# MILab-PKU/dcpt

Measured on AMD Instinct MI355X. Metric: megapixels/sec fwd+bwd NAFNet-64 256px bs=32, higher is better.
Workload: dtype f32

## Files before the change

dcpt_amd/csrc/ffn_f32.h:

```cpp
#pragma once
#include "dcpt_common.h"

struct FfnFwdF {
    const float* y;
    const float *lnw, *lnb;
    const float *W4, *W5;
    const float *b4, *b5, *gamma;
    float* out;
    float* v;
    float *mu, *rstd;
    int64_t M;
    float eps;
};
bool ffn_fwd_f32_ok(int C);
int launch_ffn_fwd_f32(const FfnFwdF& p, int C, hipStream_t s);
int launch_ln_conv_f32(const FfnFwdF& p, int C, hipStream_t s);

struct FfnBwdF {
    const float *dout, *v, *y;
    const float *wT5, *wT4;
    const float* lnw;
    float *dv, *dy;
    float* lnpart;
    int64_t M;
    float eps;
};
int ffn_bwd_f32_waves(int64_t M);
int launch_ffn_bwd_f32(const FfnBwdF& p, int C, hipStream_t s);
```

dcpt_amd/csrc/ffn_f32.hip:

```cpp
#include "bufops.h"
#include "ffn_f32.h"

namespace {

#ifdef F32_ABL_NOMFMA
#define FFN_MFMA(a, b, c) (c)
#else
#define FFN_MFMA(a, b, c) __builtin_amdgcn_mfma_f32_32x32x2f32(a, b, c, 0, 0, 0)
#endif

constexpr int FW = 4;
constexpr int S_SLOT = 8192, S_RING = 4, S_WAVE = S_RING * S_SLOT;
constexpr int S_TAB = FW * S_WAVE;
constexpr int T_B4 = 0, T_B5 = 128, T_GM = 192, T_LW = 256, T_LB = 320, T_N = 384;

__device__ __forceinline__ void lds_fence() { asm volatile("s_waitcnt lgkmcnt(0)" ::: "memory"); }

template <int C, int HEAD>
__global__ __launch_bounds__(256) void ffn_fwd_f32_kernel(const FfnFwdF p) {
    static_assert(C == 64, "ffn_fwd_f32: C = 64");
    __shared__ __attribute__((aligned(16))) unsigned char smem[S_TAB + T_N * 4];
    const int tid = threadIdx.x, lane = tid & 63;
    const int wave = __builtin_amdgcn_readfirstlane(tid >> 6);
    float* const tab = reinterpret_cast<float*>(smem + S_TAB);
    for (int i = tid; i < T_N; i += 256)
        tab[i] = i < T_B5 ? (p.b4 ? p.b4[i] : 0.f)
                          : i < T_LW ? (HEAD ? 0.f : (i < T_GM ? (p.b5 ? p.b5[i - T_B5] : 0.f) : (p.gamma ? p.gamma[i - T_GM] : 1.f)))
                                     : i < T_LB ? p.lnw[i - T_LW] : p.lnb[i - T_LB];
    const int fr = lane & 31, kh = lane >> 5;
    float W4f[4][32], W5f[2][32];
#pragma unroll
    for (int j = 0; j < 4; ++j)
#pragma unroll
        for (int q = 0; q < 8; ++q) {
// ... 113 lines not shown
#pragma unroll
            for (int j = 0; j < 2; ++j)
#pragma unroll
                for (int g = 0; g < 4; ++g) {
                    const float4 b = *reinterpret_cast<const float4*>(tab + T_B5 + 32 * j + 8 * g + 4 * kh);
                    acc2[j][4 * g + 0] = b.x; acc2[j][4 * g + 1] = b.y; acc2[j][4 * g + 2] = b.z; acc2[j][4 * g + 3] = b.w;
                }
#pragma unroll
            for (int ks = 0; ks < 32; ++ks)
#pragma unroll
                for (int j = 0; j < 2; ++j) acc2[j] = FFN_MFMA(W5f[j][ks], xf[ks], acc2[j]);
            const rsrc_t rsO = make_rsrc(p.out + r0 * C);
#pragma unroll
            for (int j = 0; j < 2; ++j)
#pragma unroll
                for (int g = 0; g < 4; ++g) {
                    const float4 gm = *reinterpret_cast<const float4*>(tab + T_GM + 32 * j + 8 * g + 4 * kh);
                    const float4 yv = yres[4 * j + g];
                    buf_st4(rsO, rowok ? (uint32_t)(fr * 256 + (8 * j + 2 * g + kh) * 16) : ROW_SENT,
                            make_float4(yv.x + acc2[j][4 * g + 0] * gm.x, yv.y + acc2[j][4 * g + 1] * gm.y, yv.z + acc2[j][4 * g + 2] * gm.z,
                                        yv.w + acc2[j][4 * g + 3] * gm.w));
                }
        }
        lds_fence();
        asm volatile("s_waitcnt vmcnt(16)" ::: "memory");
        s = (s + 1) & 3;
    }
    dma_wait_all();
}


constexpr int G_DO = 0, G_V = 4096, G_Y = 12288, G_SLOT = 16384, G_WAVE = 2 * G_SLOT;
constexpr int G_TAB = FW * G_WAVE;
typedef float floatx4v __attribute__((ext_vector_type(4)));

template <int C>
__global__ __launch_bounds__(256) void ffn_bwd_f32_kernel(const FfnBwdF p) {
    static_assert(C == 64, "ffn_bwd_f32: C = 64");
    __shared__ __attribute__((aligned(16))) unsigned char smem[G_TAB + 64 * 4];
    const int tid = threadIdx.x, lane = tid & 63;
    const int wave = __builtin_amdgcn_readfirstlane(tid >> 6);
    float* const tab = reinterpret_cast<float*>(smem + G_TAB);
    if (tid < 64) tab[tid] = p.lnw[tid];
    const int fm = lane & 15, q = lane >> 4;
    float W5f[4][16], W4f[4][32];
#pragma unroll
    for (int t = 0; t < 4; ++t) {
#pragma unroll
        for (int e = 0; e < 4; ++e) {
            const float4 w = ldg4(p.wT5 + (16 * t + fm) * C + 16 * q + 4 * e);
            W5f[t][4 * e + 0] = w.x; W5f[t][4 * e + 1] = w.y; W5f[t][4 * e + 2] = w.z; W5f[t][4 * e + 3] = w.w;
        }
#pragma unroll
        for (int e = 0; e < 8; ++e) {
            const float4 w = ldg4(p.wT4 + (16 * t + fm) * (2 * C) + 32 * q + 4 * e);
            W4f[t][4 * e + 0] = w.x; W4f[t][4 * e + 1] = w.y; W4f[t][4 * e + 2] = w.z; W4f[t][4 * e + 3] = w.w;
        }
    }
    __syncthreads();

    unsigned char* const wb = smem + wave * G_WAVE;
    const uint32_t wb_lds = lds_addr(reinterpret_cast<const float*>(wb));
    const int64_t ng = (p.M + 15) / 16;
    const int64_t wg = (int64_t)blockIdx.x * FW + wave, TW = (int64_t)gridDim.x * FW;
    auto issue = [&](int64_t gi, int s) {
        const int64_t gg = gi < ng ? gi : 0;
        const i32x4 rsD = make_rsrc_dma(p.dout + gg * (16 * C)), rsY = make_rsrc_dma(p.y + gg * (16 * C)), rsV = make_rsrc_dma(p.v + gg * (32 * C));
        const uint32_t base = wb_lds + (uint32_t)(s * G_SLOT);
#pragma unroll
        for (int pc = 0; pc < 4; ++pc) {
            const int row = 4 * pc + (lane >> 4);
            const bool ok = gi < ng && gi * 16 + row < p.M;
            const uint32_t vo = ok ? (uint32_t)(row * 256 + (((lane & 15) ^ (row & 15)) * 16)) : ROW_SENT;
            dma16(rsD, base + (uint32_t)(G_DO + pc * 1024), vo, 0);
            dma16(rsY, base + (uint32_t)(G_Y + pc * 1024), vo, 0);
        }
#pragma unroll
        for (int pc = 0; pc < 8; ++pc) {
            const int row = 2 * pc + (lane >> 5);
            const bool ok = gi < ng && gi * 16 + row < p.M;
            dma16(rsV, base + (uint32_t)(G_V + pc * 1024), ok ? (uint32_t)(row * 512 + (((lane & 31) ^ (row & 15)) * 16)) : ROW_SENT, 0);
        }
    };
    issue(wg, 0);
    issue(wg + TW, 1);
    asm volatile("s_waitcnt vmcnt(16)" ::: "memory");

    float aw[4][4], ab[4][4];
#pragma unroll
    for (int t = 0; t < 4; ++t)
#pragma unroll
        for (int r = 0; r < 4; ++r) aw[t][r] = ab[t][r] = 0.f;

    int s = 0;
    for (int64_t gi = wg; gi < ng; gi += TW) {
        unsigned char* const sl = wb + s * G_SLOT;
        const int sw = fm;
        float xb[32];
#pragma unroll
        for (int e = 0; e < 4; ++e) {
            const float4 w = *reinterpret_cast<const float4*>(sl + G_DO + fm * 256 + (((4 * q + e) ^ sw) * 16));
            xb[4 * e + 0] = w.x; xb[4 * e + 1] = w.y; xb[4 * e + 2] = w.z; xb[4 * e + 3] = w.w;
        }
        floatx4v dg[4];
#pragma unroll
        for (int t = 0; t < 4; ++t) dg[t] = floatx4v{0.f, 0.f, 0.f, 0.f};
#pragma unroll
        for (int st = 0; st < 16; ++st)
#pragma unroll
            for (int t = 0; t < 4; ++t) dg[t] = __builtin_amdgcn_mfma_f32_16x16x4f32(W5f[t][st], xb[st], dg[t], 0, 0, 0);
#pragma unroll
        for (int t = 0; t < 4; ++t) {
            float4* const a1 = reinterpret_cast<float4*>(sl + G_V + fm * 512 + (((4 * t + q) ^ sw) * 16));
            float4* const a2 = reinterpret_cast<float4*>(sl + G_V + fm * 512 + (((16 + 4 * t + q) ^ sw) * 16));
            const float4 v1 = *a1, v2 = *a2;
            const float4 d = make_float4(dg[t][0], dg[t][1], dg[t][2], dg[t][3]);
            *a1 = f4_mul(d, v2);
            *a2 = f4_mul(d, v1);
        }
        lds_fence();
#pragma unroll
        for (int e = 0; e < 8; ++e) {
            const float4 w = *reinterpret_cast<const float4*>(sl + G_V + fm * 512 + (((8 * q + e) ^ sw) * 16));
            xb[4 * e + 0] = w.x; xb[4 * e + 1] = w.y; xb[4 * e + 2] = w.z; xb[4 * e + 3] = w.w;
        }
        floatx4v dx[4];
#pragma unroll
        for (int t = 0; t < 4; ++t) dx[t] = floatx4v{0.f, 0.f, 0.f, 0.f};
#pragma unroll
        for (int st = 0; st < 32; ++st)
#pragma unroll
            for (int t = 0; t < 4; ++t) dx[t] = __builtin_amdgcn_mfma_f32_16x16x4f32(W4f[t][st], xb[st], dx[t], 0, 0, 0);
        float xh[4][4];
        float sum = 0.f;
#pragma unroll
        for (int t = 0; t < 4; ++t) {
            const float4 yv = *reinterpret_cast<const float4*>(sl + G_Y + fm * 256 + (((4 * t + q) ^ sw) * 16));
            xh[t][0] = yv.x; xh[t][1] = yv.y; xh[t][2] = yv.z; xh[t][3] = yv.w;
            sum += (yv.x + yv.y) + (yv.z + yv.w);
        }
        sum += __shfl_xor(sum, 16);
        sum += __shfl_xor(sum, 32);
        const float mean = sum * (1.0f / C);
        float sq = 0.f;
#pragma unroll
        for (int t = 0; t < 4; ++t)
#pragma unroll
            for (int r = 0; r < 4; ++r) {
                xh[t][r] -= mean;
                sq += xh[t][r] * xh[t][r];
            }
        sq += __shfl_xor(sq, 16);
        sq += __shfl_xor(sq, 32);
        const float rs = 1.0f / sqrtf(sq * (1.0f / C) + p.eps);
        const bool rowok = gi * 16 + fm < p.M;
        float s1 = 0.f, s2 = 0.f;
        float gwv[4][4];
#pragma unroll
        for (int t = 0; t < 4; ++t) {
            const float4 lw = *reinterpret_cast<const float4*>(tab + 16 * t + 4 * q);
            const float lws[4] = {lw.x, lw.y, lw.z, lw.w};
#pragma unroll
            for (int r = 0; r < 4; ++r) {
                xh[t][r] *= rs;
                const float gx = dx[t][r];
                aw[t][r] += rowok ? gx * xh[t][r] : 0.f;
                ab[t][r] += rowok ? gx : 0.f;
                const float gw = gx * lws[r];
                gwv[t][r] = gw;
                s1 += gw;
                s2 += gw * xh[t][r];
            }
        }
        s1 += __shfl_xor(s1, 16); s1 += __shfl_xor(s1, 32);
        s2 += __shfl_xor(s2, 16); s2 += __shfl_xor(s2, 32);
        s1 *= (1.0f / C);
        s2 *= (1.0f / C);
#pragma unroll
        for (int t = 0; t < 4; ++t) {
            float4* const a = reinterpret_cast<float4*>(sl + G_DO + fm * 256 + (((4 * t + q) ^ sw) * 16));
            const float4 dres = *a;
            *a = make_float4(rs * (gwv[t][0] - xh[t][0] * s2 - s1) + dres.x, rs * (gwv[t][1] - xh[t][1] * s2 - s1) + dres.y,
                             rs * (gwv[t][2] - xh[t][2] * s2 - s1) + dres.z, rs * (gwv[t][3] - xh[t][3] * s2 - s1) + dres.w);
        }
        lds_fence();
        u32x4 ody[4], odv[8];
#pragma unroll
        for (int it = 0; it < 4; ++it) {
            const int row = it * 4 + (lane >> 4), ch = lane & 15;
            ody[it] = *reinterpret_cast<const u32x4*>(sl + G_DO + row * 256 + ((ch ^ (row & 15)) * 16));
        }
#pragma unroll
        for (int it = 0; it < 8; ++it) {
            const int row = it * 2 + (lane >> 5), ch = lane & 31;
            odv[it] = *reinterpret_cast<const u32x4*>(sl + G_V + row * 512 + ((ch ^ (row & 15)) * 16));
        }
        lds_fence();
        issue(gi + 2 * TW, s);
        asm volatile("s_waitcnt vmcnt(16)" ::: "memory");
        const int64_t r0 = gi * 16;
        const rsrc_t rsO = make_rsrc(p.dy + r0 * C), rsV = make_rsrc(p.dv + r0 * (2 * C));
#pragma unroll
        for (int it = 0; it < 4; ++it) {
            const int row = it * 4 + (lane >> 4), ch = lane & 15;
            __builtin_amdgcn_raw_buffer_store_b128(ody[it], rsO, r0 + row < p.M ? (uint32_t)(row * 256 + ch * 16) : ROW_SENT, 0, 0);
        }
#pragma unroll
        for (int it = 0; it < 8; ++it) {
            const int row = it * 2 + (lane >> 5), ch = lane & 31;
            __builtin_amdgcn_raw_buffer_store_b128(odv[it], rsV, r0 + row < p.M ? (uint32_t)(row * 512 + ch * 16) : ROW_SENT, 0, 0);
        }
        s ^= 1;
    }
    dma_wait_all();
#pragma unroll
    for (int t = 0; t < 4; ++t)
#pragma unroll
        for (int r = 0; r < 4; ++r) {
            float a = aw[t][r], b = ab[t][r];
#pragma unroll
            for (int m = 1; m < 16; m <<= 1) {
                a += __shfl_xor(a, m);
                b += __shfl_xor(b, m);
            }
            if (fm == 0) {
                const int c = 16 * t + 4 * q + r;
                p.lnpart[(wg * 2 + 0) * C + c] = a;
                p.lnpart[(wg * 2 + 1) * C + c] = b;
            }
        }
}

}

bool ffn_fwd_f32_ok(int C) { return C == 64; }

static int launch(const FfnFwdF& p, int head, hipStream_t s) {
    int64_t blocks = cdiv64(cdiv64(p.M, 32), FW);
    if (blocks > 256) blocks = 256;
    if (head) ffn_fwd_f32_kernel<64, 1><<<dim3((unsigned)blocks), dim3(256), 0, s>>>(p);
    else ffn_fwd_f32_kernel<64, 0><<<dim3((unsigned)blocks), dim3(256), 0, s>>>(p);
    DCPT_CHECK_LAUNCH("ffn_fwd_f32");
    return DCPT_OK;
}

int launch_ffn_fwd_f32(const FfnFwdF& p, int C, hipStream_t s) {
    DCPT_CHECK_ARG(ffn_fwd_f32_ok(C), "ffn_fwd_f32: C=%d not supported (64)", C);
    DCPT_CHECK_ARG(p.y && p.out && p.W4 && p.W5 && p.lnw && p.lnb && p.M > 0 && (p.mu == nullptr) == (p.rstd == nullptr), "ffn_fwd_f32: null argument");
    return launch(p, 0, s);
}

int launch_ln_conv_f32(const FfnFwdF& p, int C, hipStream_t s) {
    DCPT_CHECK_ARG(ffn_fwd_f32_ok(C), "ln_conv_f32: C=%d not supported (64)", C);
    DCPT_CHECK_ARG(p.y && p.v && p.W4 && p.lnw && p.lnb && p.M > 0 && (p.mu == nullptr) == (p.rstd == nullptr), "ln_conv_f32: null argument");
    return launch(p, 1, s);
}

int ffn_bwd_f32_waves(int64_t M) {
    int64_t blocks = cdiv64(cdiv64(M, 16), FW);
    if (blocks > 256) blocks = 256;
    return (int)blocks * FW;
}

int launch_ffn_bwd_f32(const FfnBwdF& p, int C, hipStream_t s) {
    DCPT_CHECK_ARG(ffn_fwd_f32_ok(C), "ffn_bwd_f32: C=%d not supported (64)", C);
    DCPT_CHECK_ARG(p.dout && p.v && p.y && p.wT5 && p.wT4 && p.lnw && p.dv && p.dy && p.lnpart && p.M > 0, "ffn_bwd_f32: null argument");
    ffn_bwd_f32_kernel<64><<<dim3((unsigned)(ffn_bwd_f32_waves(p.M) / FW)), dim3(256), 0, s>>>(p);
    DCPT_CHECK_LAUNCH("ffn_bwd_f32");
    return DCPT_OK;
}
```

dcpt_amd/csrc/nafblock.hip:

```cpp
#include "gemm.h"
#include "kernels.h"
#include "ffn_f32.h"
#include "side.h"
#include "../../include/dcpt_hip.h"

namespace {

struct FwdWs {
    float* w2p;
    float* pool_part;
    int nblk_pool;
};

size_t fwd_ws_layout(int B, int H, int W, int C, void* base, size_t bytes, FwdWs* out) {
    WsAlloc a(base, base ? bytes : (size_t)-1);
    DwGeom g{B, H, W, C};
    const int nblk = dw_ring_usable(g, 4) ? dw_ring_num_blocks_per_image(g, 4) : dw_num_blocks_per_image(g);
    float* w2p = a.get<float>((size_t)9 * 2 * C);
    float* pp = a.get<float>((size_t)B * nblk * C);
    if (out) {
        out->w2p = w2p;
        out->pool_part = pp;
        out->nblk_pool = nblk;
    }
    return a.off;
}

struct BwdWs {
    float *wT5, *wT4, *wT3, *wT1, *w2p;
    float *b2a, *b2b, *b2c;
    float *bca, *bcb, *bcc;
    float* slab;
    float* colsum;
    size_t slab_elems, colsum_elems;
    float *lnpart, *lnpart2;
    float *ds_part, *ds, *dpool;
    float* wpart;
    int ln_nblk, nblk_b;
    float *u4, *c4, *u1, *c1, *rowpart;
    int rp_sg, rp_dw;
    float* ffn_part;
};

bool ln_in_epilogue(int C);
bool ffn_fused_f32(int C);
size_t bwd_ws_layout(int B, int H, int W, int C, void* base, size_t bytes, BwdWs* out) {
    WsAlloc a(base, base ? bytes : (size_t)-1);
    const int64_t M = (int64_t)B * H * W;
    const int P = H * W;
    DwGeom g{B, H, W, C};
    BwdWs w;
    w.wT5 = a.get<float>((size_t)C * C);
    w.wT4 = a.get<float>((size_t)2 * C * C);
    w.wT3 = a.get<float>((size_t)C * C);
    w.wT1 = a.get<float>((size_t)2 * C * C);
    w.w2p = a.get<float>((size_t)18 * C);
    w.b2a = a.get<float>((size_t)M * 2 * C);
    w.b2b = a.get<float>((size_t)M * 2 * C);
    w.b2c = a.get<float>((size_t)M * 2 * C);
    w.bca = a.get<float>((size_t)M * C);
    w.bcb = a.get<float>((size_t)M * C);
    w.bcc = a.get<float>((size_t)M * C);
    int sp1, sp2;
    int64_t r1, r2;
    gemm_tn_plan(M, 2 * C, C, &sp1, &r1);
    gemm_tn_plan(M, C, C, &sp2, &r2);
    size_t slab1 = (size_t)sp1 * 2 * C * C, slab2 = (size_t)sp2 * C * C;
    size_t cs1 = (size_t)sp1 * gemm_tn_tiles_k(2 * C, C) * 2 * C, cs2 = (size_t)sp2 * gemm_tn_tiles_k(C, C) * C;
    {
        int sp3;
        int64_t r3;
        if (gemm_tn_plan_images(M, C, C, P, &sp3, &r3)) {
            const size_t s3 = (size_t)sp3 * C * C, c3 = (size_t)sp3 * gemm_tn_tiles_k(C, C) * C;
            if (s3 > slab2) slab2 = s3;
            if (c3 > cs2) cs2 = c3;
        }
    }
    w.slab_elems = slab1 > slab2 ? slab1 : slab2;
    w.colsum_elems = cs1 > cs2 ? cs1 : cs2;
    w.slab = a.get<float>(w.slab_elems);
    w.colsum = a.get<float>(w.colsum_elems);
    w.ln_nblk = ln_bwd_num_blocks(M, C);
    {
        const size_t a1 = (size_t)w.ln_nblk * 3 * C, a2 = (size_t)cdiv64(M, 128) * 2 * C;
        w.lnpart = a.get<float>(a1 > a2 ? a1 : a2);
        w.lnpart2 = a.get<float>(a1 > a2 ? a1 : a2);
    }
    {
        const int fs = sca_ds_fused_slices(P), ns = sca_ds_num_blocks(P);
        w.ds_part = a.get<float>((size_t)B * (fs > ns ? fs : ns) * C);
    }
    w.ds = a.get<float>((size_t)B * C);
    w.dpool = a.get<float>((size_t)B * C);
    {
        const int n1 = dw_num_blocks_per_image_fused(g), n2 = dw_ring_bwd_usable(g, 4) ? dw_ring_bwd_num_blocks_per_image(g) : 0;
        w.nblk_b = n1 > n2 ? n1 : n2;
    }
    w.wpart = a.get<float>((size_t)B * w.nblk_b * 10 * 2 * C);
    w.u4 = a.get<float>((size_t)2 * C);
    w.c4 = a.get<float>((size_t)2 * C);
    w.u1 = a.get<float>((size_t)2 * C);
    w.c1 = a.get<float>((size_t)2 * C);
    w.rp_sg = cdiv(C, 64);
    w.rp_dw = dw_fused_row_chunks(g);
    w.rowpart = a.get<float>((size_t)M * (w.rp_sg > w.rp_dw ? w.rp_sg : w.rp_dw) * 2);
    w.ffn_part = ffn_fused_f32(C) ? a.get<float>((size_t)ffn_bwd_f32_waves(M) * 2 * C) : nullptr;
    if (out) *out = w;
    return a.off;
}

bool ln_rowsums(int C, int rp_sg, int rp_dw) {
    static const int on = dcpt_tuning("DCPT_LN_ROWSUMS", 0);
    return on && C > 128 && rp_sg <= 16 && rp_dw <= 16;
}

bool ffn_fused_f32(int C) {
    static const int on = dcpt_tuning("DCPT_FFN_FUSED_F32", 1);
    return on && ffn_fwd_f32_ok(C);
}

bool ln_in_epilogue(int C) {
    static const int on = dcpt_tuning("DCPT_LN_EPILOGUE", 1);
    return on && C <= 128;
}

int wgrad(const float* X, int ldx, int N, const float* Y, int ldy, int K, int yload, const GemmTN& proto, int64_t M,
          float* slab, float* colsum, const float* rowscale, const float* Wfor_gain, const float* wbias, float* dW,
          float* dgain, float* dbias, hipStream_t s) {
    GemmTN t = proto;
    t.X = X; t.ldx = ldx; t.N = N; t.Y = Y; t.ldy = ldy; t.K = K; t.M = M;
    t.slab = slab; t.colsum = colsum;
    gemm_tn_plan(M, N, K, &t.splits, &t.rows_per_split);
    DCPT_TRY(launch_gemm_tn(t, A_PLAIN, yload, s));
    DCPT_TRY(launch_wgrad_reduce(slab, colsum, t.splits, t.splits * gemm_tn_tiles_k(N, K), N, K, rowscale, Wfor_gain, wbias, dW,
                                 dgain, dbias, WR_PLAIN, s));
    return DCPT_OK;
}

}

extern "C" int dcpt_nafblock_fused_ffn(int C) { return ffn_fused_f32(C) ? 1 : 0; }
extern "C" size_t dcpt_nafblock_fwd_ws_bytes(int B, int H, int W, int C) { return fwd_ws_layout(B, H, W, C, nullptr, 0, nullptr); }
extern "C" size_t dcpt_nafblock_bwd_ws_bytes(int B, int H, int W, int C) { return bwd_ws_layout(B, H, W, C, nullptr, 0, nullptr); }

extern "C" int dcpt_nafblock_fwd(const dcpt_nafblock_params* p, const float* inp, float* out, const dcpt_nafblock_saved* sv,
                                 void* ws, size_t ws_bytes, int B, int H, int W, int C, dcpt_stream_t stream) {
    hipStream_t s = (hipStream_t)stream;
    DCPT_CHECK_ARG(p && inp && out && sv, "nafblock_fwd: null argument");
    DCPT_CHECK_ARG(B > 0 && H > 0 && W > 0 && C > 0 && C % 4 == 0, "nafblock_fwd: bad shape B=%d H=%d W=%d C=%d (C %% 4 == 0)", B, H, W, C);
    FwdWs w;
    const size_t need = fwd_ws_layout(B, H, W, C, ws, ws_bytes, &w);
// ... 74 lines not shown
    DwGeom dg{B, H, W, C};

    WpackJobs jobs{};
    jobs.n = 5;
    jobs.in[0] = p->conv5_w; jobs.out[0] = w.wT5; jobs.rs[0] = p->gamma; jobs.N[0] = C;  jobs.K[0] = C;
    jobs.in[1] = p->conv4_w; jobs.out[1] = w.wT4; jobs.rs[1] = nullptr;  jobs.N[1] = C2; jobs.K[1] = C;
    jobs.in[2] = p->conv3_w; jobs.out[2] = w.wT3; jobs.rs[2] = p->beta;  jobs.N[2] = C;  jobs.K[2] = C;
    jobs.in[3] = p->conv1_w; jobs.out[3] = w.wT1; jobs.rs[3] = nullptr;  jobs.N[3] = C2; jobs.K[3] = C;
    jobs.in[4] = p->conv2_w; jobs.out[4] = w.w2p; jobs.rs[4] = nullptr;  jobs.N[4] = C2; jobs.K[4] = 9;
    DCPT_TRY(launch_wpack_multi(jobs, s));

    float* dv = w.b2a;
    float* gln = w.bca;
    float* dy = w.bcb;
    float* dts = w.bcc;
    float* da = w.b2c;
    float* dt1 = w.b2b;
    Side* sd = side_for(s);
    hipStream_t sw = side_stream(sd, s);
    DCPT_TRY(side_fork(sd, 0, s));

    const bool lne = ln_in_epilogue(C);
    const bool lrs = !lne && ln_rowsums(C, w.rp_sg, w.rp_dw);
    if (lrs) {
        LnVecJobs lj{};
        lj.n = 2; lj.N2 = C2; lj.C = C;
        lj.W[0] = p->conv4_w; lj.bz[0] = p->conv4_b; lj.lnw[0] = p->norm2_w; lj.lnb[0] = p->norm2_b; lj.u[0] = w.u4; lj.cvec[0] = w.c4;
        lj.W[1] = p->conv1_w; lj.bz[1] = p->conv1_b; lj.lnw[1] = p->norm1_w; lj.lnb[1] = p->norm1_b; lj.u[1] = w.u1; lj.cvec[1] = w.c1;
        DCPT_TRY(launch_lnvec(lj, s));
    }
    GemmNT g{};
    GemmTN tp{};
    const bool ffn = ffn_fused_f32(C);
    int rp_b1 = 0;
    if (ffn) {
        FfnBwdF f{};
        f.dout = dout; f.v = sv->v; f.y = sv->y; f.wT5 = w.wT5; f.wT4 = w.wT4; f.lnw = p->norm2_w; f.dv = dv; f.dy = dy; f.lnpart = w.ffn_part;
        f.M = M; f.eps = 1e-6f;
        DCPT_TRY(launch_ffn_bwd_f32(f, C, s));
    } else {
        g.M = M; g.A = dout; g.lda = C; g.K = C; g.Bw = w.wT5; g.N = C; g.C = dv; g.ldc = C2; g.aux = sv->v;
        if (lrs) {
            g.rowpart = w.rowpart; g.uvec = w.u4; g.cvec = w.c4;
            rp_b1 = gemm_nt_tiles_n(g, A_PLAIN, E_SGBWD);
        }
        DCPT_TRY(launch_gemm_nt(g, A_PLAIN, E_SGBWD, s));
    }
    tp = GemmTN{};
    if (ffn) DCPT_TRY(wgrad(dout, C, C, sv->v, C2, C, A_SG, tp, M, w.slab, w.colsum, p->gamma, p->conv5_w, p->conv5_b, gr->conv5_w, gr->gamma, gr->conv5_b, sw));
    else
    DCPT_TRY(wgrad(dout, C, C, sv->g, C, C, A_PLAIN, tp, M, w.slab, w.colsum, p->gamma, p->conv5_w, p->conv5_b, gr->conv5_w,
                   gr->gamma, gr->conv5_b, sw));
    DCPT_TRY(side_fork(sd, 1, s));
    g = GemmNT{};
    const int ln_tiles = (int)cdiv64(M, 128);
    g.M = M; g.A = dv; g.lda = C2; g.K = C2; g.Bw = w.wT4; g.N = C; g.C = gln; g.ldc = C;
    if (ffn) {
    } else if (lne) {
        g.C = dy; g.res = sv->y; g.ldres = C; g.aux = dout; g.mu = sv->mu2; g.rstd = sv->rstd2; g.lnw = p->norm2_w; g.colpart = w.lnpart;
        DCPT_TRY(launch_gemm_nt(g, A_PLAIN, E_LNBWD, s));
    } else if (lrs) {
        g.C = dy; g.res = sv->y; g.ldres = C; g.aux = dout; g.mu = sv->mu2; g.rstd = sv->rstd2; g.lnw = p->norm2_w; g.colpart = w.lnpart;
        g.rowpart = w.rowpart; g.rowparts = rp_b1;
        DCPT_TRY(launch_gemm_nt(g, A_PLAIN, E_LNBWD2, s));
    } else {
        DCPT_TRY(launch_gemm_nt(g, A_PLAIN, E_PLAIN, s));
    }
    tp = GemmTN{};
    if (ffn) {
        tp.mu = sv->mu2; tp.rstd = sv->rstd2; tp.lnw = p->norm2_w; tp.lnb = p->norm2_b;
        DCPT_TRY(wgrad(dv, C2, C2, sv->y, C, C, A_LN, tp, M, w.slab, w.colsum, nullptr, nullptr, nullptr, gr->conv4_w, nullptr, gr->conv4_b, sw));
    } else
    DCPT_TRY(wgrad(dv, C2, C2, sv->xn2, C, C, A_PLAIN, tp, M, w.slab, w.colsum, nullptr, nullptr, nullptr, gr->conv4_w, nullptr,
                   gr->conv4_b, sw));
    if (!ffn && !lne && !lrs) DCPT_TRY(launch_ln_bwd(gln, sv->y, sv->mu2, sv->rstd2, p->norm2_w, dout, dy, w.lnpart, w.ln_nblk, M, C, s));
    DCPT_TRY(side_fork(sd, 2, s));
    if (ffn) DCPT_TRY(launch_colpart_reduce(w.ffn_part, ffn_bwd_f32_waves(M), 2, C, gr->norm2_w, gr->norm2_b, nullptr, sw));
    else if (lne || lrs) DCPT_TRY(launch_colpart_reduce(w.lnpart, ln_tiles, 2, C, gr->norm2_w, gr->norm2_b, nullptr, sw));
    else DCPT_TRY(launch_colpart_reduce(w.lnpart, w.ln_nblk, 3, C, gr->norm2_w, gr->norm2_b, nullptr, sw));
    const bool ds_fused = sca_ds_fused_slices(P) > 0;
    const int ds_slices = ds_fused ? sca_ds_fused_slices(P) : sca_ds_num_blocks(P);
    g = GemmNT{};
    g.M = M; g.A = dy; g.lda = C; g.K = C; g.Bw = w.wT3; g.N = C; g.C = dts; g.ldc = C;
    if (ds_fused) {
        g.res = sv->t2; g.ldres = C; g.colpart = w.ds_part;
        DCPT_TRY(launch_gemm_nt(g, A_PLAIN, E_DOTCOL, s));
    } else {
        DCPT_TRY(launch_gemm_nt(g, A_PLAIN, E_PLAIN, s));
    }
    {
        GemmTN t{};
        t.X = dy; t.ldx = C; t.N = C; t.Y = sv->t2; t.ldy = C; t.K = C; t.M = M; t.slab = w.slab; t.colsum = w.colsum;
        if (gemm_tn_plan_images(M, C, C, P, &t.splits, &t.rows_per_split) &&
            (size_t)t.splits * C * C <= w.slab_elems && (size_t)t.splits * gemm_tn_tiles_k(C, C) * C <= w.colsum_elems) {
            DCPT_TRY(launch_gemm_tn(t, A_PLAIN, A_PLAIN, sw));
            DCPT_TRY(launch_wgrad_reduce_scaled(w.slab, w.colsum, t.splits, t.splits * gemm_tn_tiles_k(C, C), C, C, p->beta, p->conv3_w,
                                                p->conv3_b, gr->conv3_w, gr->beta, gr->conv3_b, WR_PLAIN, sv->s,
                                                (int)(P / t.rows_per_split), sw));
        } else {
            tp = GemmTN{};
            tp.simg = sv->s; tp.P = P;
            DCPT_TRY(wgrad(dy, C, C, sv->t2, C, C, A_SCALE, tp, M, w.slab, w.colsum, p->beta, p->conv3_w, p->conv3_b, gr->conv3_w,
                           gr->beta, gr->conv3_b, sw));
        }
    }
    if (!ds_fused) DCPT_TRY(launch_sca_ds_part(dts, sv->t2, w.ds_part, B, C, P, s));
    DCPT_TRY(launch_sca_dpool(w.ds_part, ds_slices, p->sca_w, w.dpool, B, C, P, s));
    (void)da;
    const bool ring_b = !lrs && dw_ring_bwd_usable(dg, 4);
    const int nblk_b = ring_b ? dw_ring_bwd_num_blocks_per_image(dg) : dw_num_blocks_per_image_fused(dg);
// ... 106 lines not shown
```

Before: 18.05.

## Fuse FFN weight-gradient GEMMs into the fused f32 FFN backward kernel

Adds a WG variant of the fused FFN backward kernel. It accumulates the conv5 and conv4 weight gradients and their column sums in registers via MFMA, using the tiles already staged in LDS, and writes per-block partials. The dv intermediate is no longer written to global memory, and the two separate wgrad GEMM passes over dout/v and dv/y are skipped. A new small finish kernel folds the LayerNorm affine into dW4/db4 and computes the norm2 gradients. To make room, part of the weights moves to LDS, which raises register and LDS pressure and lengthens each iteration with extra phases and fences.

```diff
diff --git a/dcpt_amd/csrc/ffn_f32.h b/dcpt_amd/csrc/ffn_f32.h
--- a/dcpt_amd/csrc/ffn_f32.h
+++ b/dcpt_amd/csrc/ffn_f32.h
@@ -22,8 +22,12 @@
     const float* lnw;
     float *dv, *dy;
     float* lnpart;
+    float *g5, *cs5;
+    float *g4, *cs4;
     int64_t M;
     float eps;
 };
 int ffn_bwd_f32_waves(int64_t M);
 int launch_ffn_bwd_f32(const FfnBwdF& p, int C, hipStream_t s);
+int launch_ffn_ln_finish_f32(const float* G, const float* cs, const float* W4, const float* lnw, const float* lnb, float* dW4, float* db4,
+                             float* dlnw, float* dlnb, int C, hipStream_t s);
diff --git a/dcpt_amd/csrc/ffn_f32.hip b/dcpt_amd/csrc/ffn_f32.hip
--- a/dcpt_amd/csrc/ffn_f32.hip
+++ b/dcpt_amd/csrc/ffn_f32.hip
@@ -1,5 +1,6 @@
 #include "bufops.h"
 #include "ffn_f32.h"
+#include "prof.h"
 
 namespace {
 
@@ -179,27 +180,57 @@
 
 constexpr int G_DO = 0, G_V = 4096, G_Y = 12288, G_SLOT = 16384, G_WAVE = 2 * G_SLOT;
 constexpr int G_TAB = FW * G_WAVE;
+constexpr int G_W5 = G_TAB + 64 * 4, W5_LD = 68, W4_LD = 132, G_W4 = G_W5 + 64 * W5_LD * 4, W4H_LD = 68, G_W4H = G_W4 + 16 * W4_LD * 4;
+constexpr int G_END = G_W4H + 16 * W4H_LD * 4;
+static_assert(G_END <= 160 * 1024, "ffn_bwd_f32: LDS");
 typedef float floatx4v __attribute__((ext_vector_type(4)));
-
-template <int C>
+#define FFN_MFMA16(a, b, c) __builtin_amdgcn_mfma_f32_16x16x4f32(a, b, c, 0, 0, 0)
+
+#ifndef FFN_WG_PHASE_SCHED
+#define FFN_WG_PHASE_SCHED 1
+#endif
+template <int WG>
+__device__ __forceinline__ void phase_fence() {
+    lds_fence();
+#if FFN_WG_PHASE_SCHED
+    if constexpr (WG) __builtin_amdgcn_sched_barrier(0);
+#endif
+}
+
+template <int C, int WG>
 __global__ __launch_bounds__(256) void ffn_bwd_f32_kernel(const FfnBwdF p) {
     static_assert(C == 64, "ffn_bwd_f32: C = 64");
-    __shared__ __attribute__((aligned(16))) unsigned char smem[G_TAB + 64 * 4];
+    __shared__ __attribute__((aligned(16))) unsigned char smem[WG ? G_END : G_W5];
     const int tid = threadIdx.x, lane = tid & 63;
     const int wave = __builtin_amdgcn_readfirstlane(tid >> 6);
     float* const tab = reinterpret_cast<float*>(smem + G_TAB);
+    const float* const w5s = reinterpret_cast<const float*>(smem + G_W5);
+    const float* const w4s = reinterpret_cast<const float*>(smem + G_W4);
+    const float* const w4h = reinterpret_cast<const float*>(smem + G_W4H);
     if (tid < 64) tab[tid] = p.lnw[tid];
+    if constexpr (WG) {
+        for (int i = tid; i < C * C / 4; i += 256)
+            *reinterpret_cast<float4*>(smem + G_W5 + ((i >> 4) * W5_LD + 4 * (i & 15)) * 4) = ldg4(p.wT5 + 4 * i);
+        for (int i = tid; i < 16 * 2 * C / 4; i += 256)
+            *reinterpret_cast<float4*>(smem + G_W4 + ((i >> 5) * W4_LD + 4 * (i & 31)) * 4) = ldg4(p.wT4 + 4 * i);
+        *reinterpret_cast<float4*>(smem + G_W4H + ((tid >> 4) * W4H_LD + 4 * (tid & 15)) * 4) =
+            ldg4(p.wT4 + (16 + (tid >> 4)) * (2 * C) + 32 * ((tid >> 2) & 3) + 4 * (tid & 3));
+    }
     const int fm = lane & 15, q = lane >> 4;
-    float W5f[4][16], W4f[4][32];
+    constexpr int TL = WG ? 1 : 0, EH = WG ? 4 : 0;
+    float W5f[WG ? 1 : 4][16], W4f[4][32];
 #pragma unroll
     for (int t = 0; t < 4; ++t) {
-#pragma unroll
-        for (int e = 0; e < 4; ++e) {
-            const float4 w = ldg4(p.wT5 + (16 * t + fm) * C + 16 * q + 4 * e);
-            W5f[t][4 * e + 0] = w.x; W5f[t][4 * e + 1] = w.y; W5f[t][4 * e + 2] = w.z; W5f[t][4 * e + 3] = w.w;
-        }
-#pragma unroll
-        for (int e = 0; e < 8; ++e) {
+        if constexpr (!WG) {
+#pragma unroll
+            for (int e = 0; e < 4; ++e) {
+                const float4 w = ldg4(p.wT5 + (16 * t + fm) * C + 16 * q + 4 * e);
+                W5f[t][4 * e + 0] = w.x; W5f[t][4 * e + 1] = w.y; W5f[t][4 * e + 2] = w.z; W5f[t][4 * e + 3] = w.w;
+            }
+        }
+        if (t < TL) continue;
+#pragma unroll
+        for (int e = (t == TL ? EH : 0); e < 8; ++e) {
             const float4 w = ldg4(p.wT4 + (16 * t + fm) * (2 * C) + 32 * q + 4 * e);
             W4f[t][4 * e + 0] = w.x; W4f[t][4 * e + 1] = w.y; W4f[t][4 * e + 2] = w.z; W4f[t][4 * e + 3] = w.w;
         }
@@ -210,7 +241,7 @@
     const uint32_t wb_lds = lds_addr(reinterpret_cast<const float*>(wb));
     const int64_t ng = (p.M + 15) / 16;
     const int64_t wg = (int64_t)blockIdx.x * FW + wave, TW = (int64_t)gridDim.x * FW;
-    auto issue = [&](int64_t gi, int s) {
+    auto issue = [&](int64_t gi, int s, int lane) {
         const int64_t gg = gi < ng ? gi : 0;
         const i32x4 rsD = make_rsrc_dma(p.dout + gg * (16 * C)), rsY = make_rsrc_dma(p.y + gg * (16 * C)), rsV = make_rsrc_dma(p.v + gg * (32 * C));
         const uint32_t base = wb_lds + (uint32_t)(s * G_SLOT);
@@ -229,8 +260,8 @@
             dma16(rsV, base + (uint32_t)(G_V + pc * 1024), ok ? (uint32_t)(row * 512 + (((lane & 31) ^ (row & 15)) * 16)) : ROW_SENT, 0);
         }
     };
-    issue(wg, 0);
-    issue(wg + TW, 1);
+    issue(wg, 0, lane);
+    issue(wg + TW, 1, lane);
     asm volatile("s_waitcnt vmcnt(16)" ::: "memory");
 
     float aw[4][4], ab[4][4];
@@ -238,51 +269,125 @@
     for (int t = 0; t < 4; ++t)
 #pragma unroll
         for (int r = 0; r < 4; ++r) aw[t][r] = ab[t][r] = 0.f;
+    floatx4v acc5[WG ? 4 : 1][4], acc4[WG ? 8 : 1][4];
+    float cs5[4], cs4[8];
+    if constexpr (WG) {
+#pragma unroll
+        for (int i = 0; i < 4; ++i) {
+            cs5[i] = cs4[i] = cs4[i + 4] = 0.f;
+#pragma unroll
+            for (int j = 0; j < 4; ++j) acc5[i][j] = acc4[i][j] = acc4[i + 4][j] = floatx4v{0.f, 0.f, 0.f, 0.f};
+        }
+    }
 
     int s = 0;
     for (int64_t gi = wg; gi < ng; gi += TW) {
         unsigned char* const sl = wb + s * G_SLOT;
-        const int sw = fm;
+        int lanel = lane;
+        if constexpr (WG) asm volatile("" : "+v"(lanel));
+        const int fml = lanel & 15, ql = lanel >> 4;
+        const int fch = fml >> 2, fdw = (fml & 3) * 4;
+        const int sw = fml;
         float xb[32];
 #pragma unroll
         for (int e = 0; e < 4; ++e) {
-            const float4 w = *reinterpret_cast<const float4*>(sl + G_DO + fm * 256 + (((4 * q + e) ^ sw) * 16));
+            const float4 w = *reinterpret_cast<const float4*>(sl + G_DO + fml * 256 + (((4 * ql + e) ^ sw) * 16));
             xb[4 * e + 0] = w.x; xb[4 * e + 1] = w.y; xb[4 * e + 2] = w.z; xb[4 * e + 3] = w.w;
         }
         floatx4v dg[4];
+        float4 dv1[4];
 #pragma unroll
         for (int t = 0; t < 4; ++t) dg[t] = floatx4v{0.f, 0.f, 0.f, 0.f};
-#pragma unroll
-        for (int st = 0; st < 16; ++st)
-#pragma unroll
-            for (int t = 0; t < 4; ++t) dg[t] = __builtin_amdgcn_mfma_f32_16x16x4f32(W5f[t][st], xb[st], dg[t], 0, 0, 0);
+        if constexpr (WG) {
+#pragma unroll
+            for (int e = 0; e < 4; ++e) {
+                float4 w[4];
+#pragma unroll
+                for (int t = 0; t < 4; ++t) w[t] = *reinterpret_cast<const float4*>(w5s + (16 * t + fml) * W5_LD + 16 * ql + 4 * e);
+#pragma unroll
+                for (int t = 0; t < 4; ++t) {
+                    dg[t] = FFN_MFMA16(w[t].x, xb[4 * e + 0], dg[t]);
+                    dg[t] = FFN_MFMA16(w[t].y, xb[4 * e + 1], dg[t]);
+                    dg[t] = FFN_MFMA16(w[t].z, xb[4 * e + 2], dg[t]);
+                    dg[t] = FFN_MFMA16(w[t].w, xb[4 * e + 3], dg[t]);
+                }
+            }
+        } else {
+#pragma unroll
+            for (int st = 0; st < 16; ++st)
+#pragma unroll
+                for (int t = 0; t < 4; ++t) dg[t] = __builtin_amdgcn_mfma_f32_16x16x4f32(W5f[t][st], xb[st], dg[t], 0, 0, 0);
+        }
 #pragma unroll
         for (int t = 0; t < 4; ++t) {
-            float4* const a1 = reinterpret_cast<float4*>(sl + G_V + fm * 512 + (((4 * t + q) ^ sw) * 16));
-            float4* const a2 = reinterpret_cast<float4*>(sl + G_V + fm * 512 + (((16 + 4 * t + q) ^ sw) * 16));
+            float4* const a1 = reinterpret_cast<float4*>(sl + G_V + fml * 512 + (((4 * t + ql) ^ sw) * 16));
+            float4* const a2 = reinterpret_cast<float4*>(sl + G_V + fml * 512 + (((16 + 4 * t + ql) ^ sw) * 16));
             const float4 v1 = *a1, v2 = *a2;
             const float4 d = make_float4(dg[t][0], dg[t][1], dg[t][2], dg[t][3]);
-            *a1 = f4_mul(d, v2);
+            if constexpr (WG) {
+                *a1 = f4_mul(v1, v2);
+                dv1[t] = f4_mul(d, v2);
+            } else {
+                *a1 = f4_mul(d, v2);
+            }
             *a2 = f4_mul(d, v1);
         }
-        lds_fence();
+        phase_fence<WG>();
+        if constexpr (WG) {
+            float a[2][4], b[2][4];
+            auto frag5 = [&](int st) {
+                const int pm = st + 4 * ql;
+#pragma unroll
+                for (int i = 0; i < 4; ++i) {
+                    a[st & 1][i] = *reinterpret_cast<const float*>(sl + G_DO + pm * 256 + (((4 * i + fch) ^ pm) * 16) + fdw);
+                    b[st & 1][i] = *reinterpret_cast<const float*>(sl + G_V + pm * 512 + (((4 * i + fch) ^ pm) * 16) + fdw);
+                }
+            };
+            frag5(0);
+#pragma unroll
+            for (int st = 0; st < 4; ++st) {
+                if (st < 3) frag5(st + 1);
+#pragma unroll
+                for (int i = 0; i < 4; ++i) {
+                    cs5[i] += a[st & 1][i];
+#pragma unroll
+                    for (int j = 0; j < 4; ++j) acc5[i][j] = FFN_MFMA16(a[st & 1][i], b[st & 1][j], acc5[i][j]);
+                }
+                __builtin_amdgcn_sched_barrier(0);
+            }
+            phase_fence<WG>();
+#pragma unroll
+            for (int t = 0; t < 4; ++t) *reinterpret_cast<float4*>(sl + G_V + fml * 512 + (((4 * t + ql) ^ sw) * 16)) = dv1[t];
+            phase_fence<WG>();
+        }
 #pragma unroll
         for (int e = 0; e < 8; ++e) {
-            const float4 w = *reinterpret_cast<const float4*>(sl + G_V + fm * 512 + (((8 * q + e) ^ sw) * 16));
+            const float4 w = *reinterpret_cast<const float4*>(sl + G_V + fml * 512 + (((8 * ql + e) ^ sw) * 16));
             xb[4 * e + 0] = w.x; xb[4 * e + 1] = w.y; xb[4 * e + 2] = w.z; xb[4 * e + 3] = w.w;
         }
         floatx4v dx[4];
 #pragma unroll
         for (int t = 0; t < 4; ++t) dx[t] = floatx4v{0.f, 0.f, 0.f, 0.f};
 #pragma unroll
-        for (int st = 0; st < 32; ++st)
-#pragma unroll
-            for (int t = 0; t < 4; ++t) dx[t] = __builtin_amdgcn_mfma_f32_16x16x4f32(W4f[t][st], xb[st], dx[t], 0, 0, 0);
+        for (int e = 0; e < 8; ++e) {
+            float4 w[2];
+            if (TL) w[0] = *reinterpret_cast<const float4*>(w4s + fml * W4_LD + 32 * ql + 4 * e);
+            if (e < EH) w[1] = *reinterpret_cast<const float4*>(w4h + fml * W4H_LD + 16 * ql + 4 * e);
+#pragma unroll
+            for (int r = 0; r < 4; ++r)
+#pragma unroll
+                for (int t = 0; t < 4; ++t) {
+                    const bool reg = t > TL || (t == TL && e >= EH);
+                    const float wv = reg ? W4f[t][4 * e + r] : r == 0 ? w[t].x : r == 1 ? w[t].y : r == 2 ? w[t].z : w[t].w;
+                    dx[t] = FFN_MFMA16(wv, xb[4 * e + r], dx[t]);
+                }
+        }
+        if constexpr (WG) __builtin_amdgcn_sched_barrier(0);
         float xh[4][4];
         float sum = 0.f;
 #pragma unroll
         for (int t = 0; t < 4; ++t) {
-            const float4 yv = *reinterpret_cast<const float4*>(sl + G_Y + fm * 256 + (((4 * t + q) ^ sw) * 16));
+            const float4 yv = *reinterpret_cast<const float4*>(sl + G_Y + fml * 256 + (((4 * t + ql) ^ sw) * 16));
             xh[t][0] = yv.x; xh[t][1] = yv.y; xh[t][2] = yv.z; xh[t][3] = yv.w;
             sum += (yv.x + yv.y) + (yv.z + yv.w);
         }
@@ -300,21 +405,23 @@
         sq += __shfl_xor(sq, 16);
         sq += __shfl_xor(sq, 32);
         const float rs = 1.0f / sqrtf(sq * (1.0f / C) + p.eps);
-        const bool rowok = gi * 16 + fm < p.M;
+        const bool rowok = gi * 16 + fml < p.M;
         float s1 = 0.f, s2 = 0.f;
         float gwv[4][4];
 #pragma unroll
         for (int t = 0; t < 4; ++t) {
-            const float4 lw = *reinterpret_cast<const float4*>(tab + 16 * t + 4 * q);
+            const float4 lw = *reinterpret_cast<const float4*>(tab + 16 * t + 4 * ql);
             const float lws[4] = {lw.x, lw.y, lw.z, lw.w};
 #pragma unroll
             for (int r = 0; r < 4; ++r) {
                 xh[t][r] *= rs;
                 const float gx = dx[t][r];
-                aw[t][r] += rowok ? gx * xh[t][r] : 0.f;
-                ab[t][r] += rowok ? gx : 0.f;
+                if constexpr (!WG) {
+                    aw[t][r] += rowok ? gx * xh[t][r] : 0.f;
+                    ab[t][r] += rowok ? gx : 0.f;
+                }
                 const float gw = gx * lws[r];
-                gwv[t][r] = gw;
+                
                 s1 += gw;
                 s2 += gw * xh[t][r];
             }
@@ -325,57 +432,187 @@
         s2 *= (1.0f / C);
 #pragma unroll
         for (int t = 0; t < 4; ++t) {
-            float4* const a = reinterpret_cast<float4*>(sl + G_DO + fm * 256 + (((4 * t + q) ^ sw) * 16));
+            float4* const a = reinterpret_cast<float4*>(sl + G_DO + fml * 256 + (((4 * t + ql) ^ sw) * 16));
             const float4 dres = *a;
-            *a = make_float4(rs * (gwv[t][0] - xh[t][0] * s2 - s1) + dres.x, rs * (gwv[t][1] - xh[t][1] * s2 - s1) + dres.y,
-                             rs * (gwv[t][2] - xh[t][2] * s2 - s1) + dres.z, rs * (gwv[t][3] - xh[t][3] * s2 - s1) + dres.w);
-        }
-        lds_fence();
-        u32x4 ody[4], odv[8];
+            const float4 lw = *reinterpret_cast<const float4*>(tab + 16 * t + 4 * ql);
+            *a = make_float4(rs * (dx[t][0] * lw.x - xh[t][0] * s2 - s1) + dres.x, rs * (dx[t][1] * lw.y - xh[t][1] * s2 - s1) + dres.y,
+                             rs * (dx[t][2] * lw.z - xh[t][2] * s2 - s1) + dres.z, rs * (dx[t][3] * lw.w - xh[t][3] * s2 - s1) + dres.w);
+            if constexpr (WG)
+                *reinterpret_cast<float4*>(sl + G_Y + fml * 256 + (((4 * t + ql) ^ sw) * 16)) = make_float4(xh[t][0], xh[t][1], xh[t][2], xh[t][3]);
+        }
+        phase_fence<WG>();
+        if constexpr (WG) {
+            float a[2][8], b[2][4];
+            auto frag4 = [&](int st) {
+                const int pm = st + 4 * ql;
+#pragma unroll
+                for (int i = 0; i < 8; ++i) a[st & 1][i] = *reinterpret_cast<const float*>(sl + G_V + pm * 512 + (((4 * i + fch) ^ pm) * 16) + fdw);
+#pragma unroll
+                for (int j = 0; j < 4; ++j) b[st & 1][j] = *reinterpret_cast<const float*>(sl + G_Y + pm * 256 + (((4 * j + fch) ^ pm) * 16) + fdw);
+            };
+            frag4(0);
+#pragma unroll
+            for (int st = 0; st < 4; ++st) {
+                if (st < 3) frag4(st + 1);
+#pragma unroll
+                for (int i = 0; i < 8; ++i) {
+                    cs4[i] += a[st & 1][i];
+#pragma unroll
+                    for (int j = 0; j < 4; ++j) acc4[i][j] = FFN_MFMA16(a[st & 1][i], b[st & 1][j], acc4[i][j]);
+                }
+                __builtin_amdgcn_sched_barrier(0);
+            }
+        }
+        u32x4 ody[4], odv[WG ? 1 : 8];
 #pragma unroll
         for (int it = 0; it < 4; ++it) {
-            const int row = it * 4 + (lane >> 4), ch = lane & 15;
+            const int row = it * 4 + (lanel >> 4), ch = lanel & 15;
             ody[it] = *reinterpret_cast<const u32x4*>(sl + G_DO + row * 256 + ((ch ^ (row & 15)) * 16));
         }
-#pragma unroll
-        for (int it = 0; it < 8; ++it) {
-            const int row = it * 2 + (lane >> 5), ch = lane & 31;
-            odv[it] = *reinterpret_cast<const u32x4*>(sl + G_V + row * 512 + ((ch ^ (row & 15)) * 16));
-        }
-        lds_fence();
-        issue(gi + 2 * TW, s);
+        if constexpr (!WG) {
+#pragma unroll
+            for (int it = 0; it < 8; ++it) {
+                const int row = it * 2 + (lanel >> 5), ch = lanel & 31;
+                odv[it] = *reinterpret_cast<const u32x4*>(sl + G_V + row * 512 + ((ch ^ (row & 15)) * 16));
+            }
+        }
+        phase_fence<WG>();
+        issue(gi + 2 * TW, s, lanel);
         asm volatile("s_waitcnt vmcnt(16)" ::: "memory");
         const int64_t r0 = gi * 16;
-        const rsrc_t rsO = make_rsrc(p.dy + r0 * C), rsV = make_rsrc(p.dv + r0 * (2 * C));
+        const rsrc_t rsO = make_rsrc(p.dy + r0 * C);
 #pragma unroll
         for (int it = 0; it < 4; ++it) {
-            const int row = it * 4 + (lane >> 4), ch = lane & 15;
+            const int row = it * 4 + (lanel >> 4), ch = lanel & 15;
             __builtin_amdgcn_raw_buffer_store_b128(ody[it], rsO, r0 + row < p.M ? (uint32_t)(row * 256 + ch * 16) : ROW_SENT, 0, 0);
         }
-#pragma unroll
-        for (int it = 0; it < 8; ++it) {
-            const int row = it * 2 + (lane >> 5), ch = lane & 31;
-            __builtin_amdgcn_raw_buffer_store_b128(odv[it], rsV, r0 + row < p.M ? (uint32_t)(row * 512 + ch * 16) : ROW_SENT, 0, 0);
+        if constexpr (!WG) {
+            const rsrc_t rsV = make_rsrc(p.dv + r0 * (2 * C));
+#pragma unroll
+            for (int it = 0; it < 8; ++it) {
+                const int row = it * 2 + (lanel >> 5), ch = lanel & 31;
+                __builtin_amdgcn_raw_buffer_store_b128(odv[it], rsV, r0 + row < p.M ? (uint32_t)(row * 512 + ch * 16) : ROW_SENT, 0, 0);
+            }
         }
         s ^= 1;
     }
     dma_wait_all();
-#pragma unroll
-    for (int t = 0; t < 4; ++t)
-#pragma unroll
-        for (int r = 0; r < 4; ++r) {
-            float a = aw[t][r], b = ab[t][r];
-#pragma unroll
-            for (int m = 1; m < 16; m <<= 1) {
-                a += __shfl_xor(a, m);
-                b += __shfl_xor(b, m);
-            }
-            if (fm == 0) {
-                const int c = 16 * t + 4 * q + r;
-                p.lnpart[(wg * 2 + 0) * C + c] = a;
-                p.lnpart[(wg * 2 + 1) * C + c] = b;
-            }
-        }
+    const int lanee = WG ? (int)__builtin_amdgcn_mbcnt_hi(~0u, __builtin_amdgcn_mbcnt_lo(~0u, 0u)) : lane, fme = lanee & 15, qe = lanee >> 4;
+    if constexpr (!WG) {
+#pragma unroll
+        for (int t = 0; t < 4; ++t)
+#pragma unroll
+            for (int r = 0; r < 4; ++r) {
+                float a = aw[t][r], b = ab[t][r];
+#pragma unroll
+                for (int m = 1; m < 16; m <<= 1) {
+                    a += __shfl_xor(a, m);
+                    b += __shfl_xor(b, m);
+                }
+                if (fme == 0) {
+                    const int c = 16 * t + 4 * qe + r;
+                    p.lnpart[(wg * 2 + 0) * C + c] = a;
+                    p.lnpart[(wg * 2 + 1) * C + c] = b;
+                }
+            }
+    }
+    if constexpr (WG) {
+#pragma unroll
+        for (int i = 0; i < 4; ++i) {
+            cs5[i] += __shfl_xor(cs5[i], 16); cs5[i] += __shfl_xor(cs5[i], 32);
+            cs4[i] += __shfl_xor(cs4[i], 16); cs4[i] += __shfl_xor(cs4[i], 32);
+            cs4[i + 4] += __shfl_xor(cs4[i + 4], 16); cs4[i + 4] += __shfl_xor(cs4[i + 4], 32);
+        }
+        float* const ex = reinterpret_cast<float*>(smem) + lanee;
+        __syncthreads();
+#pragma unroll 1
+        for (int w = 1; w < FW; ++w) {
+            if (wave == w) {
+#pragma unroll
+                for (int i = 0; i < 4; ++i)
+#pragma unroll
+                    for (int j = 0; j < 4; ++j)
+#pragma unroll
+                        for (int r = 0; r < 4; ++r) {
+                            ex[(16 * i + 4 * j + r) * 64] = acc5[i][j][r];
+                            ex[(64 + 16 * i + 4 * j + r) * 64] = acc4[i][j][r];
+                            ex[(128 + 16 * i + 4 * j + r) * 64] = acc4[i + 4][j][r];
+                        }
+#pragma unroll
+                for (int i = 0; i < 4; ++i) {
+                    ex[(192 + i) * 64] = cs5[i];
+                    ex[(196 + i) * 64] = cs4[i];
+                    ex[(200 + i) * 64] = cs4[i + 4];
+                }
+            }
+            __syncthreads();
+            if (wave == 0) {
+#pragma unroll
+                for (int i = 0; i < 4; ++i)
+#pragma unroll
+                    for (int j = 0; j < 4; ++j)
+#pragma unroll
+                        for (int r = 0; r < 4; ++r) {
+                            acc5[i][j][r] += ex[(16 * i + 4 * j + r) * 64];
+                            acc4[i][j][r] += ex[(64 + 16 * i + 4 * j + r) * 64];
+                            acc4[i + 4][j][r] += ex[(128 + 16 * i + 4 * j + r) * 64];
+                        }
+#pragma unroll
+                for (int i = 0; i < 4; ++i) {
+                    cs5[i] += ex[(192 + i) * 64];
+                    cs4[i] += ex[(196 + i) * 64];
+                    cs4[i + 4] += ex[(200 + i) * 64];
+                }
+            }
+            __syncthreads();
+        }
+        if (wave == 0) {
+            float* const g5 = p.g5 + (int64_t)blockIdx.x * (C * C) + fme;
+            float* const g4 = p.g4 + (int64_t)blockIdx.x * (2 * C * C) + fme;
+#pragma unroll
+            for (int i = 0; i < 4; ++i)
+#pragma unroll
+                for (int j = 0; j < 4; ++j)
+#pragma unroll
+                    for (int r = 0; r < 4; ++r) {
+                        g5[(16 * i + 4 * qe + r) * C + 16 * j] = acc5[i][j][r];
+                        g4[(16 * i + 4 * qe + r) * C + 16 * j] = acc4[i][j][r];
+                        g4[(64 + 16 * i + 4 * qe + r) * C + 16 * j] = acc4[i + 4][j][r];
+                    }
+            if (qe == 0) {
+#pragma unroll
+                for (int i = 0; i < 4; ++i) {
+                    p.cs5[(int64_t)blockIdx.x * C + 16 * i + fme] = cs5[i];
+                    p.cs4[(int64_t)blockIdx.x * (2 * C) + 16 * i + fme] = cs4[i];
+                    p.cs4[(int64_t)blockIdx.x * (2 * C) + 64 + 16 * i + fme] = cs4[i + 4];
+                }
+            }
+        }
+    }
+}
+
+template <int C>
+__global__ __launch_bounds__(256) void ffn_ln_finish_kernel(const float* __restrict__ G, const float* __restrict__ cs, const float* __restrict__ W4,
+                                                            const float* __restrict__ lnw, const float* __restrict__ lnb, float* __restrict__ dW4,
+                                                            float* __restrict__ db4, float* __restrict__ dlnw, float* __restrict__ dlnb) {
+    __shared__ float red[2][4][C];
+    const int tid = threadIdx.x, c = tid & (C - 1), jq = tid / C;
+    const float lw = lnw[c], lb = lnb[c];
+    float aw = 0.f, ab = 0.f;
+    for (int j = jq; j < 2 * C; j += 256 / C) {
+        const float g = G[j * C + c], sj = cs[j], w = W4[j * C + c];
+        dW4[j * C + c] = g * lw + sj * lb;
+        aw += w * g;
+        ab += w * sj;
+    }
+    red[0][jq][c] = aw;
+    red[1][jq][c] = ab;
+    if (tid < 2 * C) db4[tid] = cs[tid];
+    __syncthreads();
+    if (tid < C) {
+        dlnw[tid] = (red[0][0][tid] + red[0][1][tid]) + (red[0][2][tid] + red[0][3][tid]);
+        dlnb[tid] = (red[1][0][tid] + red[1][1][tid]) + (red[1][2][tid] + red[1][3][tid]);
+    }
 }
 
 }
@@ -411,8 +648,22 @@
 
 int launch_ffn_bwd_f32(const FfnBwdF& p, int C, hipStream_t s) {
     DCPT_CHECK_ARG(ffn_fwd_f32_ok(C), "ffn_bwd_f32: C=%d not supported (64)", C);
-    DCPT_CHECK_ARG(p.dout && p.v && p.y && p.wT5 && p.wT4 && p.lnw && p.dv && p.dy && p.lnpart && p.M > 0, "ffn_bwd_f32: null argument");
-    ffn_bwd_f32_kernel<64><<<dim3((unsigned)(ffn_bwd_f32_waves(p.M) / FW)), dim3(256), 0, s>>>(p);
+    DCPT_CHECK_ARG(p.dout && p.v && p.y && p.wT5 && p.wT4 && p.lnw && p.dy && p.M > 0, "ffn_bwd_f32: null argument");
+    const bool wg = p.g5 != nullptr;
+    DCPT_CHECK_ARG(wg ? (p.g4 && p.cs5 && p.cs4) : (p.dv && p.lnpart && !p.g4 && !p.cs5 && !p.cs4), "ffn_bwd_f32: dv and lnpart, or all of g5 / cs5 / g4 / cs4");
+    const dim3 grid((unsigned)(ffn_bwd_f32_waves(p.M) / FW));
+    trace_tag(wg ? "ffn64f.bwd_wgrad" : "ffn64f.bwd");
+    if (wg) ffn_bwd_f32_kernel<64, 1><<<grid, dim3(256), 0, s>>>(p);
+    else ffn_bwd_f32_kernel<64, 0><<<grid, dim3(256), 0, s>>>(p);
     DCPT_CHECK_LAUNCH("ffn_bwd_f32");
     return DCPT_OK;
 }
+
+int launch_ffn_ln_finish_f32(const float* G, const float* cs, const float* W4, const float* lnw, const float* lnb, float* dW4, float* db4,
+                             float* dlnw, float* dlnb, int C, hipStream_t s) {
+    DCPT_CHECK_ARG(ffn_fwd_f32_ok(C), "ffn_ln_finish_f32: C=%d not supported (64)", C);
+    DCPT_CHECK_ARG(G && cs && W4 && lnw && lnb && dW4 && db4 && dlnw && dlnb, "ffn_ln_finish_f32: null argument");
+    ffn_ln_finish_kernel<64><<<dim3(1), dim3(256), 0, s>>>(G, cs, W4, lnw, lnb, dW4, db4, dlnw, dlnb);
+    DCPT_CHECK_LAUNCH("ffn_ln_finish_f32");
+    return DCPT_OK;
+}
diff --git a/dcpt_amd/csrc/nafblock.hip b/dcpt_amd/csrc/nafblock.hip
--- a/dcpt_amd/csrc/nafblock.hip
+++ b/dcpt_amd/csrc/nafblock.hip
@@ -40,10 +40,12 @@
     float *u4, *c4, *u1, *c1, *rowpart;
     int rp_sg, rp_dw;
     float* ffn_part;
+    float *ffn_g5, *ffn_cs5, *ffn_g4, *ffn_cs4, *ffn_g4t, *ffn_cs4t;
 };
 
 bool ln_in_epilogue(int C);
 bool ffn_fused_f32(int C);
+bool ffn_wgrad_f32(int C);
 size_t bwd_ws_layout(int B, int H, int W, int C, void* base, size_t bytes, BwdWs* out) {
     WsAlloc a(base, base ? bytes : (size_t)-1);
     const int64_t M = (int64_t)B * H * W;
@@ -105,6 +107,16 @@
     w.rp_dw = dw_fused_row_chunks(g);
     w.rowpart = a.get<float>((size_t)M * (w.rp_sg > w.rp_dw ? w.rp_sg : w.rp_dw) * 2);
     w.ffn_part = ffn_fused_f32(C) ? a.get<float>((size_t)ffn_bwd_f32_waves(M) * 2 * C) : nullptr;
+    w.ffn_g5 = w.ffn_cs5 = w.ffn_g4 = w.ffn_cs4 = w.ffn_g4t = w.ffn_cs4t = nullptr;
+    if (ffn_wgrad_f32(C)) {
+        const size_t nb = (size_t)ffn_bwd_f32_waves(M) / 4;
+        w.ffn_g5 = a.get<float>(nb * C * C);
+        w.ffn_cs5 = a.get<float>(nb * C);
+        w.ffn_g4 = a.get<float>(nb * 2 * C * C);
+        w.ffn_cs4 = a.get<float>(nb * 2 * C);
+        w.ffn_g4t = a.get<float>((size_t)2 * C * C);
+        w.ffn_cs4t = a.get<float>((size_t)2 * C);
+    }
     if (out) *out = w;
     return a.off;
 }
@@ -117,6 +129,11 @@
 bool ffn_fused_f32(int C) {
     static const int on = dcpt_tuning("DCPT_FFN_FUSED_F32", 1);
     return on && ffn_fwd_f32_ok(C);
+}
+
+bool ffn_wgrad_f32(int C) {
+    static const int on = dcpt_tuning("DCPT_FFN_WGRAD_F32", 1);
+    return on && ffn_fused_f32(C);
 }
 
 bool ln_in_epilogue(int C) {
@@ -257,10 +274,17 @@
     GemmNT g{};
     GemmTN tp{};
     const bool ffn = ffn_fused_f32(C);
+    const bool ffw = ffn_wgrad_f32(C);
+    const int ffn_nb = ffn ? ffn_bwd_f32_waves(M) / 4 : 0;
     int rp_b1 = 0;
     if (ffn) {
         FfnBwdF f{};
-        f.dout = dout; f.v = sv->v; f.y = sv->y; f.wT5 = w.wT5; f.wT4 = w.wT4; f.lnw = p->norm2_w; f.dv = dv; f.dy = dy; f.lnpart = w.ffn_part;
+        f.dout = dout; f.v = sv->v; f.y = sv->y; f.wT5 = w.wT5; f.wT4 = w.wT4; f.lnw = p->norm2_w; f.dy = dy;
+        if (ffw) {
+            f.g5 = w.ffn_g5; f.cs5 = w.ffn_cs5; f.g4 = w.ffn_g4; f.cs4 = w.ffn_cs4;
+        } else {
+            f.dv = dv; f.lnpart = w.ffn_part;
+        }
         f.M = M; f.eps = 1e-6f;
         DCPT_TRY(launch_ffn_bwd_f32(f, C, s));
     } else {
@@ -272,7 +296,8 @@
         DCPT_TRY(launch_gemm_nt(g, A_PLAIN, E_SGBWD, s));
     }
     tp = GemmTN{};
-    if (ffn) DCPT_TRY(wgrad(dout, C, C, sv->v, C2, C, A_SG, tp, M, w.slab, w.colsum, p->gamma, p->conv5_w, p->conv5_b, gr->conv5_w, gr->gamma, gr->conv5_b, sw));
+    if (ffw) {
+    } else if (ffn) DCPT_TRY(wgrad(dout, C, C, sv->v, C2, C, A_SG, tp, M, w.slab, w.colsum, p->gamma, p->conv5_w, p->conv5_b, gr->conv5_w, gr->gamma, gr->conv5_b, sw));
     else
     DCPT_TRY(wgrad(dout, C, C, sv->g, C, C, A_PLAIN, tp, M, w.slab, w.colsum, p->gamma, p->conv5_w, p->conv5_b, gr->conv5_w,
                    gr->gamma, gr->conv5_b, sw));
@@ -292,7 +317,8 @@
         DCPT_TRY(launch_gemm_nt(g, A_PLAIN, E_PLAIN, s));
     }
     tp = GemmTN{};
-    if (ffn) {
+    if (ffw) {
+    } else if (ffn) {
         tp.mu = sv->mu2; tp.rstd = sv->rstd2; tp.lnw = p->norm2_w; tp.lnb = p->norm2_b;
         DCPT_TRY(wgrad(dv, C2, C2, sv->y, C, C, A_LN, tp, M, w.slab, w.colsum, nullptr, nullptr, nullptr, gr->conv4_w, nullptr, gr->conv4_b, sw));
     } else
@@ -300,7 +326,13 @@
                    gr->conv4_b, sw));
     if (!ffn && !lne && !lrs) DCPT_TRY(launch_ln_bwd(gln, sv->y, sv->mu2, sv->rstd2, p->norm2_w, dout, dy, w.lnpart, w.ln_nblk, M, C, s));
     DCPT_TRY(side_fork(sd, 2, s));
-    if (ffn) DCPT_TRY(launch_colpart_reduce(w.ffn_part, ffn_bwd_f32_waves(M), 2, C, gr->norm2_w, gr->norm2_b, nullptr, sw));
+    if (ffw) {
+        DCPT_TRY(launch_wgrad_reduce(w.ffn_g5, w.ffn_cs5, ffn_nb, ffn_nb, C, C, p->gamma, p->conv5_w, p->conv5_b, gr->conv5_w, gr->gamma, gr->conv5_b,
+                                     WR_PLAIN, sw));
+        DCPT_TRY(launch_wgrad_reduce(w.ffn_g4, w.ffn_cs4, ffn_nb, ffn_nb, C2, C, nullptr, nullptr, nullptr, w.ffn_g4t, nullptr, w.ffn_cs4t, WR_PLAIN, sw));
+        DCPT_TRY(launch_ffn_ln_finish_f32(w.ffn_g4t, w.ffn_cs4t, p->conv4_w, p->norm2_w, p->norm2_b, gr->conv4_w, gr->conv4_b, gr->norm2_w, gr->norm2_b,
+                                          C, sw));
+    } else if (ffn) DCPT_TRY(launch_colpart_reduce(w.ffn_part, ffn_bwd_f32_waves(M), 2, C, gr->norm2_w, gr->norm2_b, nullptr, sw));
     else if (lne || lrs) DCPT_TRY(launch_colpart_reduce(w.lnpart, ln_tiles, 2, C, gr->norm2_w, gr->norm2_b, nullptr, sw));
     else DCPT_TRY(launch_colpart_reduce(w.lnpart, w.ln_nblk, 3, C, gr->norm2_w, gr->norm2_b, nullptr, sw));
     const bool ds_fused = sca_ds_fused_slices(P) > 0;
```

New measurement: 18.17 (median of 6 runs). No clear change (+0.6%).
